# z430/keyword-spotting

Hardware: AMD Instinct MI355X
Metric: 1s 16kHz clips/sec end-to-end (wav->label) (higher is better)
Workload: dtype f32

## Files before the change

keyword-spotting_amd/csrc/kws_dscnn.hip:

```cpp
#include <type_traits>

#include "kws_internal.h"
#include "kws_mfcc_dev.h"
#include "kws_split_mfma.h"

namespace kws {
namespace {


#ifndef KWS_DSCNN_WAVES
#define KWS_DSCNN_WAVES 8
#endif
#ifndef KWS_X_DSCNN_STAMP_TID
#define KWS_X_DSCNN_STAMP_TID 0
#endif
constexpr int NW = KWS_DSCNN_WAVES;
constexpr int NT = NW * 64;
constexpr int TW = 30;

constexpr int P0 = C1_H * C1_W;
constexpr int FEAT_H = 103, FEAT_W = 14;
constexpr int OFF_Z3 = 0, OFF_Z2 = 22976, OFF_Z1 = 0, OFF_Z0 = 9152, OFF_FEAT = 18304;
constexpr int OFF_DWTAB = 38784;
constexpr int OFF_PWB = OFF_DWTAB + 2 * 768;
// ... 69 lines not shown
struct DwPair {
    float4 l[5];
};
template <bool TO_MFMA, int E>
__device__ __forceinline__ float stencil3x3_of_pair(const DwPair& w, float up, float mid, float dn, float mask_l, float mask_r) {
    if constexpr (E == 0)
        return stencil3x3<TO_MFMA>(w.l[0].x, w.l[0].z, w.l[1].x, w.l[1].z, w.l[2].x, w.l[2].z, w.l[3].x, w.l[3].z, w.l[4].x, w.l[4].z, up, mid, dn,
                                   mask_l, mask_r);
    else
        return stencil3x3<TO_MFMA>(w.l[0].y, w.l[0].w, w.l[1].y, w.l[1].w, w.l[2].y, w.l[2].w, w.l[3].y, w.l[3].w, w.l[4].y, w.l[4].w, up, mid, dn,
                                   mask_l, mask_r);
}
__device__ __forceinline__ float half_wave_sum_to_last_lane(float v) {
    v = dpp_shift_add<0x111, 0xf>(v);
    v = dpp_shift_add<0x112, 0xf>(v);
    v = dpp_shift_add<0x114, 0xf>(v);
    v = dpp_shift_add<0x118, 0xf>(v);
    v = dpp_shift_add<0x142, 0xa>(v);
    return v;
}

struct BlockTables {
    float d0, d1, b;
};
__device__ __forceinline__ void fetch_block_tables(const DscnnWeights& w, int n, int tid, BlockTables& r) {
    const float* src = w.dw_w + (n - 1) * CH * 12;
    r.d0 = tid < CH * 12 ? src[tid] : 0.f;
    r.d1 = NT + tid < CH * 12 ? src[NT + tid] : 0.f;
    r.b = tid < CH ? w.pw_b[(n - 1) * CH + tid] : 0.f;
}
__device__ __forceinline__ void store_block_tables(float* lds, int n, int tid, const BlockTables& r, float s_dwb = 1.f, float s_pwb = 1.f,
                                                   float s_dww = 1.f) {
    float* dwtab = lds + OFF_DWTAB + ((n - 1) & 1) * 768;
    if (tid < CH * 12) dwtab[tid] = r.d0 * ((tid % 24) >> 1 == 9 ? s_dwb : s_dww);
    if (NT + tid < CH * 12) dwtab[NT + tid] = r.d1 * (((NT + tid) % 24) >> 1 == 9 ? s_dwb : s_dww);
    if (tid < CH) lds[OFF_PWB + ((n - 1) & 1) * 64 + tid] = r.b * s_pwb;
}
struct PairCtx {
    float s_dww = 1.f;
    float s_dwb = 1.f;
    float s_pwb = 1.f;
    float inv_out = 1.f;
};
__device__ __forceinline__ void cap_units(int& ky, int& sg, int k_w, float bz) {
    sg = ky + k_w;
    const int eb = (int)((__builtin_bit_cast(uint32_t, bz) >> 23) & 0xffu) - 126;
    int limit = 100 - eb;
    limit = limit > 120 ? 120 : limit;
    if (sg > limit) {
        ky -= sg - limit;
        sg = limit;
    }
}
__device__ __forceinline__ void publish_wave_max(float* lds, int set, int wv, int lane, float mx) {
    auto step = [](float m, auto ctrl, auto row_mask) {
        return fmaxf(m, __builtin_bit_cast(float, __builtin_amdgcn_update_dpp(__builtin_bit_cast(int, m), __builtin_bit_cast(int, m), decltype(ctrl)::value,
                                                                              decltype(row_mask)::value, 0xf, false)));
    };
    mx = step(mx, std::integral_constant<int, 0x111>{}, std::integral_constant<int, 0xf>{});
    mx = step(mx, std::integral_constant<int, 0x112>{}, std::integral_constant<int, 0xf>{});
    mx = step(mx, std::integral_constant<int, 0x114>{}, std::integral_constant<int, 0xf>{});
    mx = step(mx, std::integral_constant<int, 0x118>{}, std::integral_constant<int, 0xf>{});
    mx = step(mx, std::integral_constant<int, 0x142>{}, std::integral_constant<int, 0xa>{});
    mx = step(mx, std::integral_constant<int, 0x143>{}, std::integral_constant<int, 0xc>{});
    if (lane == 63) lds[OFF_WMAX + set * NW + wv] = mx;
}
__device__ __forceinline__ float read_stage_max(const float* lds, int set0, int n_sets) {
    static_assert(NW % 4 == 0 && OFF_WMAX % 4 == 0, "the stage maxima are read as float4s");
    float m = 0.f;
    const float4* q = reinterpret_cast<const float4*>(lds + OFF_WMAX + set0 * NW);
    for (int i = 0; i < (NW / 4) * n_sets; ++i) {
        const float4 v = q[i];
        m = fmaxf(fmaxf(m, fmaxf(v.x, v.y)), fmaxf(v.z, v.w));
    }
    return m;
}

template <int NP>
struct PwRing {
    uintx4 ring[2][2][NP];
};
struct PwRegsF32 {
    float wa[2][32];
};
template <int MODE>
using PwOperands = std::conditional_t<(MODE >= 4), PwRing<(MODE == 5 ? 2 : 3)>, PwRegsF32>;
__device__ __forceinline__ void load_pointwise(const DscnnWeights& w, int n, int lane, PwRegsF32& o) {
    const float* pw = w.pw_w + (n - 1) * CH * CH + 8 * (lane >> 5) * CH + (lane & 31);
#pragma unroll
    for (int ct = 0; ct < 2; ++ct)
#pragma unroll
        for (int s = 0; s < 32; ++s) o.wa[ct][s] = pw[(16 * (s >> 3) + (s & 7)) * CH + ct * 32];
}
template <int NP>
__device__ __forceinline__ void load_afrag(const DscnnWeights& w, int n, int m, int lane, uintx4 (&f)[2][NP]) {
    const uintx4* src = reinterpret_cast<const uintx4*>(NP == 2 ? w.pw_pair : w.pw_split) + (size_t)(n - 1) * (2 * 4 * NP * 64) + lane;
#pragma unroll
    for (int ct = 0; ct < 2; ++ct)
#pragma unroll
        for (int p = 0; p < NP; ++p) f[ct][p] = src[((ct * 4 + m) * NP + p) * 64];
}
__device__ __forceinline__ void load_block_head(const DscnnWeights& w, int n, int lane, PwRegsF32& o) { load_pointwise(w, n, lane, o); }
template <int NP>
__device__ __forceinline__ void load_block_head(const DscnnWeights& w, int n, int lane, PwRing<NP>& o) { load_afrag(w, n, 0, lane, o.ring[0]); }

template <bool MFMA>
__device__ __forceinline__ void conv1_phase(const DscnnWeights& w, float* lds, int tid, const float (&a)[50]) {
    const float* featp = lds + OFF_FEAT;
    float* z0 = lds + OFF_Z0;
    if constexpr (MFMA) {
        const int lane = tid & 63, wv = tid >> 6, half = lane >> 5, col = lane & 31;
        const int ct = wv & 1;
        for (int u = wv; u < 10; u += NW) {
            const int pt = u >> 1;
            const int pos = pt * 32 + col;
            const int posc = pos < P0 ? pos : P0 - 1;
            const int oh = posc / C1_W, ow = posc % C1_W;
// ... 118 lines not shown
                __builtin_amdgcn_sched_barrier(0);
            }
            if (kb + 3 < 7) gather(kb + 3, y[nxt]);
            __builtin_amdgcn_sched_barrier(0);
            product(2);
        } else {
#pragma unroll
            for (int i = 0; i < 4; ++i) {
                product(i);
                if (kb + 1 < 7) {
                    const float a0 = y[nxt][2 * i], a1 = y[nxt][2 * i + 1];
                    const float r0 = a0 - top16(a0), r1 = a1 - top16(a1);
                    bf[nxt][0][i] = pack_top16(a0, a1);
                    bf[nxt][1][i] = pack_top16(r0, r1);
                    bf[nxt][NP - 1][i] = pack_top16(r0 - top16(r0), r1 - top16(r1));
                    __builtin_amdgcn_sched_barrier(0);
                }
            }
            product(4);
            if (kb + 3 < 7) gather(kb + 3, y[nxt]);
            __builtin_amdgcn_sched_barrier(0);
            product(5);
        }
        if (DUAL && kb + 2 < 7) {
            load_other(kb + 2);
            __builtin_amdgcn_sched_barrier(0);
        }
    }
    acc += acc2;
    occ += occ2;
    if (pos < p_hi) {
#pragma unroll
        for (int r = 0; r < 16; r += 2) {
            const int co = ct * 32 + row_of(r, half);
            const float v0 = relu(fmaf(w.c1_b[co], sig0, acc[r])), v1 = relu(fmaf(w.c1_b[co + 1], sig0, acc[r + 1]));
            *reinterpret_cast<float2*>(z0 + pidx(co, pos, P0 + 2)) = make_float2(v0, v1);
            if constexpr (PAIR) mx = fmaxf(mx, fmaxf(v0, v1));
            if (DUAL) {
                const int oo = (ct ^ 1) * 32 + row_of(r, half);
                const float u0 = relu(fmaf(w.c1_b[oo], sig0, occ[r])), u1 = relu(fmaf(w.c1_b[oo + 1], sig0, occ[r + 1]));
                *reinterpret_cast<float2*>(z0 + pidx(oo, pos, P0 + 2)) = make_float2(u0, u1);
                if constexpr (PAIR) mx = fmaxf(mx, fmaxf(u0, u1));
            }
        }
    }
}

constexpr int C1W_ROWS = FEAT_H;
constexpr int OFF_C1W8 = OFF_Z1;
constexpr int OFF_C1P2 = OFF_C1W8 + 2 * C1W_ROWS * 3 * 4;
static_assert(OFF_C1P2 + 2 * C1W_ROWS * 3 <= OFF_Z0, "conv1's operand windows live where block 1's output goes later");
static_assert(2 * (C1_W - 1) + 9 < FEAT_W && 2 * (C1_H - 1) + 9 < FEAT_H, "window reach inside the padded map");

__device__ __forceinline__ void conv1_build_windows(float* lds, int tid, float sx, int off_feat = OFF_FEAT) {
    const float* featp = lds + off_feat;
    uint32_t* w8 = reinterpret_cast<uint32_t*>(lds + OFF_C1W8);
    uint32_t* p2 = reinterpret_cast<uint32_t*>(lds + OFF_C1P2);
    for (int i = tid; i < C1W_ROWS * 3; i += NT) {
        const float* src = featp + (i / 3) * FEAT_W + 2 * (i % 3);
        const float y[8] = {src[0], src[1], src[2], src[3], src[4], src[5], src[6], src[7]};
        uintx4 hi, lo;
        split_pair8(y, sx, hi, lo);
        *reinterpret_cast<uintx4*>(w8 + i * 4) = hi;
        *reinterpret_cast<uintx4*>(w8 + (C1W_ROWS * 3 + i) * 4) = lo;
        uint32_t h, l;
        split_pair2(src[8], src[9], sx, h, l);
        p2[i] = h;
        p2[C1W_ROWS * 3 + i] = l;
    }
}

template <bool DUAL>
__device__ __forceinline__ void conv1_unit_pairwin(const DscnnWeights& w, const float* lds, float* z0, int ptile, int ct, int lane,
                                                   const uintx4 (&c1f)[7][2], int p_lo, int p_hi, float sig0, float& mx) {
    const int half = lane >> 5, col = lane & 31;
    const int pos = p_lo + ptile * 32 + col;
    const int posc = pos < p_hi ? pos : p_hi - 1;
    const int oh = posc / C1_W, ow = posc % C1_W;
    const int wi = (2 * oh + 5 * half) * 3 + ow;
    const uintx4* w8 = reinterpret_cast<const uintx4*>(lds + OFF_C1W8) + wi;
    const uint32_t* p2 = reinterpret_cast<const uint32_t*>(lds + OFF_C1P2) + wi;
    const floatx16 zero = {0, 0, 0, 0, 0, 0, 0, 0, 0, 0, 0, 0, 0, 0, 0, 0};
    floatx16 acc = zero, acc2 = zero, occ = zero, occ2 = zero;
    const uintx4* osrc = reinterpret_cast<const uintx4*>(w.c1_pair) + (size_t)(ct ^ 1) * (7 * 2 * 64) + lane;
    uintx4 of[DUAL ? 7 : 1][2];
    if (DUAL) {
#pragma unroll
        for (int kb = 0; kb < 7; ++kb) {
            of[kb][0] = osrc[(kb * 2 + 0) * 64];
            of[kb][1] = osrc[(kb * 2 + 1) * 64];
        }
    }
    float4 cb[4], ob[DUAL ? 4 : 1];
#pragma unroll
    for (int q = 0; q < 4; ++q) {
        cb[q] = *reinterpret_cast<const float4*>(w.c1_b + ct * 32 + 8 * q + 4 * half);
        if (DUAL) ob[DUAL ? q : 0] = *reinterpret_cast<const float4*>(w.c1_b + (ct ^ 1) * 32 + 8 * q + 4 * half);
    }
    uintx4 bq[3][2];
    auto b_load = [&](int kb, uintx4 (&d)[2]) {
        if (kb < 5) {
            d[0] = w8[kb * 3];
            d[1] = w8[kb * 3 + C1W_ROWS * 3];
        } else if (kb == 5) {
#pragma unroll
            for (int i = 0; i < 4; ++i) {
                d[0][i] = p2[i * 3];
                d[1][i] = p2[i * 3 + C1W_ROWS * 3];
            }
        } else {
            d[0] = uintx4{p2[4 * 3], 0u, 0u, 0u};
            d[1] = uintx4{p2[4 * 3 + C1W_ROWS * 3], 0u, 0u, 0u};
        }
    };
    b_load(0, bq[0]);
    b_load(1, bq[1]);
#pragma unroll
    for (int kb = 0; kb < 7; ++kb) {
        if (kb + 2 < 7) b_load(kb + 2, bq[(kb + 2) % 3]);
        const uintx4 &bh = bq[kb % 3][0], &bl = bq[kb % 3][1];
        acc2 = mfma_f16(c1f[kb][0], bl, acc2);
        if (DUAL) occ2 = mfma_f16(of[DUAL ? kb : 0][0], bl, occ2);
        acc = mfma_f16(c1f[kb][1], bh, acc);
        if (DUAL) occ = mfma_f16(of[DUAL ? kb : 0][1], bh, occ);
        acc2 = mfma_f16(c1f[kb][0], bh, acc2);
        if (DUAL) occ2 = mfma_f16(of[DUAL ? kb : 0][0], bh, occ2);
    }
    acc += acc2;
    occ += occ2;
    if (pos < p_hi) {
#pragma unroll
        for (int r = 0; r < 16; r += 2) {
            const int co = ct * 32 + row_of(r, half);
            const float4 b4 = cb[r >> 2];
            const float b0 = (r & 2) ? b4.z : b4.x, b1 = (r & 2) ? b4.w : b4.y;
            const float v0 = relu(fmaf(b0, sig0, acc[r])), v1 = relu(fmaf(b1, sig0, acc[r + 1]));
            *reinterpret_cast<float2*>(z0 + pidx(co, pos, P0 + 2)) = make_float2(v0, v1);
            mx = fmaxf(mx, fmaxf(v0, v1));
            if (DUAL) {
                const int oo = (ct ^ 1) * 32 + row_of(r, half);
                const float4 o4 = ob[DUAL ? (r >> 2) : 0];
                const float c0 = (r & 2) ? o4.z : o4.x, c1 = (r & 2) ? o4.w : o4.y;
                const float u0 = relu(fmaf(c0, sig0, occ[r])), u1 = relu(fmaf(c1, sig0, occ[r + 1]));
                *reinterpret_cast<float2*>(z0 + pidx(oo, pos, P0 + 2)) = make_float2(u0, u1);
                mx = fmaxf(mx, fmaxf(u0, u1));
            }
        }
    }
}

struct PosRange {
    int lo, hi;
};

template <bool RANGED, int NP>
__device__ __forceinline__ void conv1_phase_split(const DscnnWeights& w, float* lds, int tid, const uintx4 (&c1f)[7][NP],
                                                  PosRange rg, float sx = 1.f, float sig0 = 1.f, int off_feat = OFF_FEAT) {
    static_assert(P0 > 4 * 32 && P0 <= 5 * 32 && NW >= 6, "conv1 work split: four dual tiles + one tile in two halves");
    const float* featp = lds + off_feat;
    float* z0 = lds + OFF_Z0;
    const int lane = tid & 63, wv = tid >> 6;
    float mx = 0.f;
    if constexpr (NP == 2) {
        if constexpr (RANGED) {
            const int n_pt = (rg.hi - rg.lo + 31) / 32;
            for (int u = wv; u < 2 * n_pt; u += NW) conv1_unit_pairwin<false>(w, lds, z0, u >> 1, u & 1, lane, c1f, rg.lo, rg.hi, sig0, mx);
        } else if (wv < 4)
            conv1_unit_pairwin<true>(w, lds, z0, wv, wv & 1, lane, c1f, 0, P0, sig0, mx);
        else if (wv < 6)
            conv1_unit_pairwin<false>(w, lds, z0, 4, wv & 1, lane, c1f, 0, P0, sig0, mx);
    } else if constexpr (RANGED) {
        const int n_pt = (rg.hi - rg.lo + 31) / 32;
        for (int u = wv; u < 2 * n_pt; u += NW) conv1_unit_split<false, NP>(w, featp, z0, u >> 1, u & 1, lane, c1f, rg.lo, rg.hi, sx, sig0, mx);
    } else if (wv < 4)
        conv1_unit_split<true, NP>(w, featp, z0, wv, wv & 1, lane, c1f, 0, P0, sx, sig0, mx);
    else if (wv < 6)
        conv1_unit_split<false, NP>(w, featp, z0, 4, wv & 1, lane, c1f, 0, P0, sx, sig0, mx);
    if constexpr (NP == 2) publish_wave_max(lds, 1, wv, lane, mx);
    if (tid < CH) {
        z0[pidx(tid, P0, P0 + 2)] = 0.f;
        z0[pidx(tid, P0 + 1, P0 + 2)] = 0.f;
    }
}

template <int N, int NP>
__device__ __forceinline__ void leftover_partial_unit(float* lds, int lane, int M, const uintx4 (&af)[2][NP]) {
    using G = Blk<N>;
    using L = Leftover<N>;
    const int half = lane >> 5, col = lane & 31;
    const float* dwtab = lds + OFF_DWTAB + G::BUF * 768;
    const float4* dwt4 = reinterpret_cast<const float4*>(dwtab) + half * 24;
    const int pos = L::P0T - 1 + col;
    const bool valid = col >= 1 && col <= TW && pos < G::POUT;
    const int posc = pos < G::POUT ? pos : G::POUT - 1;
    const int h = posc / G::W, x = posc % G::W;
    const float mask_l = x > 0 ? 1.f : 0.f, mask_r = x < G::W - 1 ? 1.f : 0.f;
    int ta[3];
#pragma unroll
    for (int dh = -1; dh <= 1; ++dh) {
        const int o = G::RING ? 1 : 0;
        const int hh = h + dh - o, xx = x - o;
        const bool inside = (unsigned)hh < (unsigned)G::HI && (unsigned)xx < (unsigned)G::WI;
        const bool in_map = (unsigned)(h + dh) < (unsigned)G::H;
        const int a = inside ? hh * G::WI + xx : ((G::RING && in_map) ? G::PIN : G::PIN + 1);
        ta[dh + 1] = G::OFF_IN + pidx(half * 8, a, G::SIN);
    }
    float y[8];
#pragma unroll
    for (int j = 0; j < 8; j += 2) {
        const int cs = 16 * M + j;
        const int o = cs * G::SIN;
        const float2 up = *reinterpret_cast<const float2*>(lds + ta[0] + o);
        const float2 mid = *reinterpret_cast<const float2*>(lds + ta[1] + o);
        const float2 dn = *reinterpret_cast<const float2*>(lds + ta[2] + o);
        DwPair wp;
#pragma unroll
        for (int i = 0; i < 5; ++i) wp.l[i] = dwt4[(cs >> 1) * 6 + i];
        y[j] = stencil3x3_of_pair<false, 0>(wp, up.x, mid.x, dn.x, mask_l, mask_r);
        y[j + 1] = stencil3x3_of_pair<false, 1>(wp, up.y, mid.y, dn.y, mask_l, mask_r);
    }
    floatx16 acc0 = {0, 0, 0, 0, 0, 0, 0, 0, 0, 0, 0, 0, 0, 0, 0, 0}, acc1 = acc0;
    if constexpr (NP == 2) {
        uintx4 bh, bl;
// ... 420 lines not shown
                    "v_add_f32_dpp %8, %8, %8 row_bcast:15 row_mask:0xa bank_mask:0xf\n\t"
                    "v_add_f32_dpp %9, %9, %9 row_bcast:15 row_mask:0xa bank_mask:0xf\n\t"
                    "v_add_f32_dpp %10, %10, %10 row_bcast:15 row_mask:0xa bank_mask:0xf\n\t"
                    "v_add_f32_dpp %11, %11, %11 row_bcast:15 row_mask:0xa bank_mask:0xf\n\t"
                    "v_add_f32_dpp %12, %12, %12 row_bcast:15 row_mask:0xa bank_mask:0xf\n\t"
                    "v_add_f32_dpp %13, %13, %13 row_bcast:15 row_mask:0xa bank_mask:0xf\n\t"
                    "v_add_f32_dpp %14, %14, %14 row_bcast:15 row_mask:0xa bank_mask:0xf\n\t"
                    "v_add_f32_dpp %15, %15, %15 row_bcast:15 row_mask:0xa bank_mask:0xf"
                    : "+v"(q[0]), "+v"(q[1]), "+v"(q[2]), "+v"(q[3]), "+v"(q[4]), "+v"(q[5]), "+v"(q[6]), "+v"(q[7]), "+v"(q[8]), "+v"(q[9]), "+v"(q[10]), "+v"(q[11]), "+v"(q[12]), "+v"(q[13]), "+v"(q[14]), "+v"(q[15]));
            }
            if (col == 31) {
#pragma unroll
                for (int k = 0; k < 32; ++k) poolbuf[wv * CH + (k >> 4) * 32 + row_of(k & 15, half)] = psum[k >> 4][k & 15] * pc.inv_out;
            }
        }
    }
    (void)bias4;
}

template <int NP>
__device__ __forceinline__ void load_conv1_frags(const DscnnWeights& w, int wv, int lane, uintx4 (&c1f)[7][NP]) {
    const uintx4* src = reinterpret_cast<const uintx4*>(NP == 2 ? w.c1_pair : w.c1_split) + (size_t)(wv & 1) * (7 * NP * 64) + lane;
#pragma unroll
    for (int kb = 0; kb < 7; ++kb)
#pragma unroll
        for (int p = 0; p < NP; ++p) c1f[kb][p] = src[(kb * NP + p) * 64];
}

__device__ __forceinline__ int wave_argmax_first(float v, int lane, int C) {
    float m = v;
    m = fmaxf(m, __builtin_bit_cast(float, __builtin_amdgcn_update_dpp(__builtin_bit_cast(int, m), __builtin_bit_cast(int, m), 0x111, 0xf, 0xf, false)));
    m = fmaxf(m, __builtin_bit_cast(float, __builtin_amdgcn_update_dpp(__builtin_bit_cast(int, m), __builtin_bit_cast(int, m), 0x112, 0xf, 0xf, false)));
    m = fmaxf(m, __builtin_bit_cast(float, __builtin_amdgcn_update_dpp(__builtin_bit_cast(int, m), __builtin_bit_cast(int, m), 0x114, 0xf, 0xf, false)));
    m = fmaxf(m, __builtin_bit_cast(float, __builtin_amdgcn_update_dpp(__builtin_bit_cast(int, m), __builtin_bit_cast(int, m), 0x118, 0xf, 0xf, false)));
    m = fmaxf(m, __builtin_bit_cast(float, __builtin_amdgcn_update_dpp(__builtin_bit_cast(int, m), __builtin_bit_cast(int, m), 0x142, 0xa, 0xf, false)));
    m = fmaxf(m, __builtin_bit_cast(float, __builtin_amdgcn_update_dpp(__builtin_bit_cast(int, m), __builtin_bit_cast(int, m), 0x143, 0xc, 0xf, false)));
    const float vmax = __builtin_bit_cast(float, __builtin_amdgcn_readlane(__builtin_bit_cast(int, m), 63));
    const unsigned long long holders = __ballot(lane < C && v == vmax);
    return holders ? __ffsll(holders) - 1 : 0;
}

__device__ __forceinline__ DscnnWeights weights_for_this_clip() {
#if defined(__HIP_DEVICE_COMPILE__)
    using KArg = const __attribute__((address_space(4))) DscnnWeights*;
    KArg p = (KArg)__builtin_amdgcn_kernarg_segment_ptr();
    asm volatile("" : "+s"(p));
    return *p;
#else
    return DscnnWeights{};
#endif
}

template <bool PAIR>
__device__ __forceinline__ void stage_features_persist(float* lds, const float* __restrict__ feat, int clip, int tid) {
    constexpr int ST = STAGE_WAVES * 64;
    constexpr int FV = (IN_T * IN_F + ST - 1) / ST;
    static_assert(2 * STAGE_WAVES == NW, "each staging wavefront zeroes the maximum slot of one other wavefront");
    const int lane = tid & 63, wv = tid >> 6;
    const float* f = feat + (size_t)clip * (IN_T * IN_F);
    float fv[FV];
#pragma unroll
    for (int k = 0; k < FV; ++k) {
        const int i = tid + k * ST;
        fv[k] = i < IN_T * IN_F ? f[i] : 0.f;
    }
    float* featp = lds + OFF_FEAT_P;
    for (int i = tid; i < FEAT_H * FEAT_W; i += ST) {
        const int r = i / FEAT_W - 2, c = i % FEAT_W - 2;
        if (!((unsigned)r < (unsigned)IN_T && (unsigned)c < (unsigned)IN_F)) featp[i] = 0.f;
    }
#pragma unroll
    for (int k = 0; k < FV; ++k) {
        const int i = tid + k * ST;
        if (i < IN_T * IN_F) featp[(i / IN_F + 2) * FEAT_W + (i % IN_F) + 2] = fv[k];
    }
    if constexpr (PAIR) {
        float m = 0.f;
#pragma unroll
        for (int k = 0; k < FV; ++k) m = fmaxf(m, fabsf(fv[k]));
        publish_wave_max(lds, 0, wv, lane, m);
        if (lane == 63) lds[OFF_WMAX + wv + STAGE_WAVES] = 0.f;
    }
}

__device__ __forceinline__ void pool_fc_wave(const DscnnWeights& w, const float* lds, int lane, int clip, float* __restrict__ logits,
                                             int32_t* __restrict__ label, float* __restrict__ a_pool) {
    const int C = w.num_classes;
    float4 fcw[CH / 4];
    float fcb = 0.f;
    const float4* wr = reinterpret_cast<const float4*>(w.fc_w + (lane < C ? lane : 0) * CH);
#pragma unroll
    for (int c = 0; c < CH / 4; ++c) fcw[c] = wr[c];
    if (lane < C) fcb = w.fc_b[lane];
    const float ring_b = w.pw_b[3 * CH + lane];
    constexpr float RING_N = 55.f * 11.f - 53.f * 9.f;
    float s = 0.f;
#pragma unroll
    for (int k = 0; k < NW; ++k) s += lds[OFF_POOLBUF_P + k * CH + lane];
    s = fmaf(RING_N, relu(ring_b), s) * (1.0f / (55.f * 11.f));
    if (a_pool) a_pool[lane] = s;
    float acc = fcb;
#pragma unroll
    for (int c = 0; c < CH / 4; ++c) {
        const float4 a4 = fcw[c];
        acc = fmaf(a4.x, __builtin_bit_cast(float, __builtin_amdgcn_readlane(__builtin_bit_cast(int, s), 4 * c + 0)), acc);
        acc = fmaf(a4.y, __builtin_bit_cast(float, __builtin_amdgcn_readlane(__builtin_bit_cast(int, s), 4 * c + 1)), acc);
        acc = fmaf(a4.z, __builtin_bit_cast(float, __builtin_amdgcn_readlane(__builtin_bit_cast(int, s), 4 * c + 2)), acc);
        acc = fmaf(a4.w, __builtin_bit_cast(float, __builtin_amdgcn_readlane(__builtin_bit_cast(int, s), 4 * c + 3)), acc);
    }
    if (lane < C) logits[(size_t)clip * C + lane] = acc;
    const int idx = wave_argmax_first(lane < C ? acc : -INFINITY, lane, C);
    if (label && lane == 0) label[clip] = idx;
}


template <int MODE, bool DIAG = true, bool PRECONV = false, bool STREAM = false, bool CLUSTER = false, bool PERSIST = false>
__global__ __launch_bounds__(NT) void kws_dscnn_fwd_kernel(DscnnWeights w_arg, const float* __restrict__ feat, int B,
                                                           float* __restrict__ logits, int32_t* __restrict__ label,
                                                           float* __restrict__ act_arg,
                                                           unsigned long long* __restrict__ stamps_arg,
                                                           const int* __restrict__ ring_hops, StreamPush sp) {
    static_assert(!STREAM || (MODE >= 4 && !DIAG && !PRECONV), "the fused push exists for the product paths only");
    static_assert(!PERSIST || ((MODE == 4 || MODE == 5) && !PRECONV && !STREAM), "persistent workgroups: batched product paths only");
    constexpr bool PAIR = MODE == 5;
    constexpr int NP = PAIR ? 2 : 3;
    BlockTables t1_pre{};
    static_assert(!CLUSTER || STREAM, "time-tile clusters exist for the streaming push only");
    float* const act = DIAG ? act_arg : nullptr;
    unsigned long long* const stamps = DIAG ? stamps_arg : nullptr;
    extern __shared__ __attribute__((aligned(16))) float lds[];
    constexpr bool MFMA = MODE != 0;
    const int tid_k = threadIdx.x;
    const int lane_k = tid_k & 63, wv_k = tid_k >> 6;

    const int cl_n = CLUSTER ? sp.cluster : 1;
    int clip = CLUSTER ? (int)blockIdx.x / cl_n : (int)blockIdx.x;
    const int cl_tile = CLUSTER ? (int)blockIdx.x - clip * cl_n : 0;
    if (clip >= B) return;
    const int j0 = Blk<4>::H * cl_tile / cl_n, j1 = Blk<4>::H * (cl_tile + 1) / cl_n;
    auto rows = [&](int lo, int hi, int H, int W) { return PosRange{(lo < 0 ? 0 : lo) * W, (hi > H ? H : hi) * W}; };
    const PosRange rg4 = rows(j0, j1, Blk<4>::H, Blk<4>::W), rg3 = rows(j0 - 2, j1, Blk<3>::H, Blk<3>::W),
                   rg2 = rows(j0 - 4, j1, Blk<2>::H, Blk<2>::W), rg1 = rows(j0 - 6, j1, Blk<1>::H, Blk<1>::W),
                   rg0 = rows(j0 - 7, j1 + 1, C1_H, C1_W);
    int n_stamp = 0;
    auto stamp = [&]() {
        if (stamps && tid_k == KWS_X_DSCNN_STAMP_TID) stamps[(size_t)clip * KWS_DSCNN_STAMPS + n_stamp] = __builtin_amdgcn_s_memtime();
        ++n_stamp;
    };

    constexpr bool SPLIT = MODE >= 4;
    BlockTables t1p{};
    uintx4 c1p[PERSIST ? 7 : 1][NP];
    int prev_clip = -1;
    float* a_prev = nullptr;
    if constexpr (PERSIST) {
        fetch_block_tables(w_arg, 1, tid_k, t1p);
        if (wv_k < STAGE_WAVES) stage_features_persist<PAIR>(lds, feat, clip, tid_k);
        load_conv1_frags(w_arg, wv_k, lane_k, c1p);
        __syncthreads();
    }
    for (;;) {
    const DscnnWeights w = PERSIST ? weights_for_this_clip() : w_arg;
    int tid = tid_k;
    if constexpr (PERSIST) {
        int wv_l = __builtin_amdgcn_readfirstlane(wv_k), lane_l = lane_k;
        asm volatile("" : "+s"(wv_l), "+v"(lane_l));
        tid = (wv_l << 6) | (lane_l & 63);
    }
    const int lane = tid & 63, wv = tid >> 6;
    if constexpr (PERSIST) n_stamp = 0;
    if (stamps && tid == KWS_X_DSCNN_STAMP_TID) stamps[(size_t)clip * KWS_DSCNN_STAMPS + KWS_DSCNN_STAMPS - 2] = __builtin_amdgcn_s_memrealtime();
    stamp();

    PwOperands<MODE> wa;
    int hops_before = 0;
    int kx = 0, ky[5] = {0, 0, 0, 0, 0}, sg[5] = {0, 0, 0, 0, 0};
    if constexpr (PERSIST) {
        if constexpr (PAIR) {
            const float mxf = read_stage_max(lds, 0, 1);
            kx = pow2_exp_for(mxf);
            const float bz0 = (w.c1_abs * mxf + w.c1_bmax) * 1.001f;
            cap_units(kx, sg[0], w.k_c1, bz0);
            const float by1 = (w.dw_abs[0] * bz0 + w.dw_bmax[0]) * 1.001f;
            ky[1] = pow2_exp_for(by1);
            cap_units(ky[1], sg[1], w.k_pw[0], (w.pw_abs[0] * by1 + w.pw_bmax[0]) * 1.001f);
            store_block_tables(lds, 1, tid, t1p, pow2f(ky[1]), pow2f(sg[1]), pow2f(ky[1] - sg[0]));
            conv1_build_windows(lds, tid, pow2f(kx), OFF_FEAT_P);
            __syncthreads();
        } else {
            store_block_tables(lds, 1, tid, t1p);
        }
        stamp();
        conv1_phase_split<false, NP>(w, lds, tid, c1p, rg0, pow2f(kx), pow2f(sg[0]), OFF_FEAT_P);
        if (wv == NW - 1 && prev_clip >= 0) {
            pool_fc_wave(w, lds, lane, prev_clip, logits, label, a_prev);
            if (stamps && lane == 0) stamps[(size_t)prev_clip * KWS_DSCNN_STAMPS + 13] = __builtin_amdgcn_s_memtime();
        }
        load_afrag(w, 1, wv >= 4 ? wv - 4 : 0, lane, wa.ring[0]);
    } else if constexpr (PRECONV) {
        static_assert(!PRECONV || MODE >= 4, "the pre-convolved entry exists for the product (split) path only");
        const float* z = feat + (size_t)clip * (CH * P0);
        fetch_block_tables(w, 1, tid, t1_pre);
        float zmax = 0.f;
        for (int i = tid; i < CH * P0; i += NT) {
            const float v = z[i];
            lds[OFF_Z0 + pidx(i / P0, i % P0, P0 + 2)] = v;
            zmax = fmaxf(zmax, v);
        }
        if (tid < CH) {
            lds[OFF_Z0 + pidx(tid, P0, P0 + 2)] = 0.f;
            lds[OFF_Z0 + pidx(tid, P0 + 1, P0 + 2)] = 0.f;
        }
        if constexpr (PAIR)
            publish_wave_max(lds, 1, wv, lane, zmax);
        else
            store_block_tables(lds, 1, tid, t1_pre);
        if constexpr (Leftover<1>::HAS && (MODE == 4 || MODE == 5) && !CLUSTER)
            load_afrag(w, 1, wv >= 4 ? wv - 4 : 0, lane, wa.ring[0]);
        else
            load_block_head(w, 1, lane, wa);
        stamp();
    } else {
    float* featp = lds + OFF_FEAT;
    const float* f = feat + (size_t)clip * (IN_T * IN_F);
    constexpr int FV = (IN_T * IN_F + NT - 1) / NT;
    float fv[FV];
    int row_new = -1;
    int head;
    if constexpr (STREAM) {
        hops_before = *sp.hops;
        const int K = (sp.p.frame_len + sp.p.frame_step - 1) / sp.p.frame_step;
        head = (((hops_before + 2 - K) % IN_T) + IN_T) % IN_T;
        const int step = sp.p.frame_step;
        const long f_start = (long)step * hops_before + step - (long)((sp.p.frame_len + step - 1) / step) * step;
        if (f_start >= 0) row_new = (int)((((f_start / step) - head) % IN_T + IN_T) % IN_T);
    } else {
        head = ring_hops ? (((*ring_hops + 1 - sp.frames_lag) % IN_T) + IN_T) % IN_T : 0;
    }
#pragma unroll
    for (int k = 0; k < FV; ++k) {
        const int i = tid + k * NT;
        fv[k] = (i < IN_T * IN_F && i / IN_F != row_new) ? f[((i / IN_F + head) % IN_T) * IN_F + i % IN_F] : 0.f;
    }
    BlockTables t1;
    fetch_block_tables(w, 1, tid, t1);
    __builtin_amdgcn_sched_barrier(0);
// ... 121 lines not shown
    if constexpr (PAIR) {
        const float mz = fmaxf(read_stage_max(lds, 2, (Leftover<1>::HAS && KSL_ON) ? 2 : 1) * pow2f(-sg[1]), w.pw_bmax[0]);
        const float bz = (w.pw_abs[1] * ((w.dw_abs[1] * mz + w.dw_bmax[1]) * 1.001f) + w.pw_bmax[1]) * 1.001f;
        const float by = (w.dw_abs[2] * bz + w.dw_bmax[2]) * 1.001f;
        ky[3] = pow2_exp_for(by);
        cap_units(ky[3], sg[3], w.k_pw[2], (w.pw_abs[2] * by + w.pw_bmax[2]) * 1.001f);
        pc.s_dww = pow2f(ky[3] - sg[2]);
        pc.s_dwb = pow2f(ky[3]);
        pc.s_pwb = pow2f(sg[3]);
    }
    block_phase<2, MODE, CLUSTER>(w, lds, tid, wa, nullptr, rg2, pc);
    stamp();
    __syncthreads();
    if constexpr (Leftover<2>::HAS && KSL_ON) {
        leftover_combine<2, PAIR>(lds, tid);
        __syncthreads();
    }
    stamp();
    if (a) {
        const float u = PAIR ? pow2f(-sg[2]) : 1.f;
        for (int i = tid; i < CH * Blk<2>::POUT; i += NT)
            a[i] = lds[OFF_Z2 + pidx(i / Blk<2>::POUT, i % Blk<2>::POUT, Blk<2>::SOUT)] * u;
        a += CH * Blk<2>::POUT;
    }
    if constexpr (PAIR) {
        const float mz = fmaxf(read_stage_max(lds, 0, (Leftover<2>::HAS && KSL_ON) ? 2 : 1) * pow2f(-sg[2]), w.pw_bmax[1]);
        const float bz = (w.pw_abs[2] * ((w.dw_abs[2] * mz + w.dw_bmax[2]) * 1.001f) + w.pw_bmax[2]) * 1.001f;
        const float by = (w.dw_abs[3] * bz + w.dw_bmax[3]) * 1.001f;
        ky[4] = pow2_exp_for(by);
        cap_units(ky[4], sg[4], w.k_pw[3], (w.pw_abs[3] * by + w.pw_bmax[3]) * 1.001f);
        pc.s_dww = pow2f(ky[4] - sg[3]);
        pc.s_dwb = pow2f(ky[4]);
        pc.s_pwb = pow2f(sg[4]);
    }
    block_phase<3, MODE, CLUSTER>(w, lds, tid, wa, nullptr, rg3, pc);
    stamp();
    __syncthreads();
    stamp();
    if (a) {
        const float u = PAIR ? pow2f(-sg[3]) : 1.f;
        for (int i = tid; i < CH * Blk<3>::POUT; i += NT)
            a[i] = lds[OFF_Z3 + pidx(i / Blk<3>::POUT, i % Blk<3>::POUT, Blk<3>::SOUT)] * u;
        a += CH * Blk<3>::POUT;
    }
    if constexpr (PAIR) {
        pc.inv_out = pow2f(-sg[4]);
    }
    block_phase<4, MODE, CLUSTER>(w, lds, tid, wa, a ? a + CH : nullptr, rg4, pc,
                                  PERSIST ? OFF_POOLBUF_P : OFF_POOLBUF);
    stamp();
    if constexpr (PERSIST) {
        const int next = clip + (int)gridDim.x;
        __builtin_amdgcn_sched_barrier(0);
        if (wv < STAGE_WAVES && next < B) stage_features_persist<PAIR>(lds, feat, next, tid);
        stamp();
        load_conv1_frags(w, wv, lane, c1p);
        __syncthreads();
        stamp();
        if (stamps && tid == KWS_X_DSCNN_STAMP_TID) stamps[(size_t)clip * KWS_DSCNN_STAMPS + KWS_DSCNN_STAMPS - 1] = __builtin_amdgcn_s_memrealtime();
        prev_clip = clip;
        a_prev = a;
        clip = next;
        if (clip >= B) break;
        continue;
    }
    const int C = w.num_classes;
    float4 fcw[CH / 4];
    float fcb = 0.f, ring_b = 0.f;
    if (wv == 0 && lane < C) {
        const float4* wr = reinterpret_cast<const float4*>(w.fc_w + lane * CH);
#pragma unroll
        for (int c = 0; c < CH / 4; ++c) fcw[c] = wr[c];
        fcb = w.fc_b[lane];
    }
    if (tid < CH) ring_b = w.pw_b[3 * CH + tid];
    __syncthreads();
    stamp();

    float* pooled = lds + OFF_POOLED;
    constexpr float RING_N = 55.f * 11.f - 53.f * 9.f;
    bool run_fc = true;
    if constexpr (CLUSTER) {
        float* part = sp.cl_part + ((size_t)clip * cl_n + cl_tile) * CH;
        if (tid < CH) {
            float s = 0.f;
#pragma unroll
            for (int k = 0; k < NW; ++k) s += lds[OFF_POOLBUF + k * CH + tid];
            __hip_atomic_store(part + tid, s, __ATOMIC_RELAXED, __HIP_MEMORY_SCOPE_AGENT);
        }
        asm volatile("s_waitcnt vmcnt(0)" ::: "memory");
        __syncthreads();
        int* last_flag = reinterpret_cast<int*>(lds + OFF_POOLED + CH);
        if (tid == 0) {
            const int arrived = atomicAdd(&sp.cl_count[clip], 1);
            *last_flag = arrived == cl_n - 1;
            if (arrived == cl_n - 1) sp.cl_count[clip] = 0;
        }
        __syncthreads();
        run_fc = *last_flag != 0;
        if (run_fc) {
            if (tid < CH) {
                float s = 0.f;
                for (int t = 0; t < cl_n; ++t)
                    s += __hip_atomic_load(sp.cl_part + ((size_t)clip * cl_n + t) * CH + tid, __ATOMIC_RELAXED, __HIP_MEMORY_SCOPE_AGENT);
                pooled[tid] = fmaf(RING_N, relu(ring_b), s) * (1.0f / (55.f * 11.f));
            }
        }
// ... 326 lines not shown
```

Baseline: 7.050 million.

## Build next clip's conv1 windows and block-1 tables during the previous clip's tail

In the persistent kernel, the staging wavefronts now compute the next clip's input maximum, derive the front scale exponents, write the block-1 depthwise and pointwise tables, and build the split conv1 operand windows straight from global memory into a spare region of the Z2 plane. This removes the per-clip table fetch/store, the window build, and one __syncthreads from the head of each clip, and drops the padded feature staging on the pair path. In exchange, the staging waves do more global loads and more arithmetic in the tail, including a redundant per-wave read of the full clip for the max. The change also relies on new LDS overlap invariants, which are asserted statically.

```diff
diff --git a/keyword-spotting_amd/csrc/kws_dscnn.hip b/keyword-spotting_amd/csrc/kws_dscnn.hip
--- a/keyword-spotting_amd/csrc/kws_dscnn.hip
+++ b/keyword-spotting_amd/csrc/kws_dscnn.hip
@@ -145,7 +145,15 @@
         sg = limit;
     }
 }
-__device__ __forceinline__ void publish_wave_max(float* lds, int set, int wv, int lane, float mx) {
+__device__ __forceinline__ void front_scales(const DscnnWeights& w, float mxf, int& kx, int& sg0, int& ky1, int& sg1) {
+    kx = pow2_exp_for(mxf);
+    const float bz0 = (w.c1_abs * mxf + w.c1_bmax) * 1.001f;
+    cap_units(kx, sg0, w.k_c1, bz0);
+    const float by1 = (w.dw_abs[0] * bz0 + w.dw_bmax[0]) * 1.001f;
+    ky1 = pow2_exp_for(by1);
+    cap_units(ky1, sg1, w.k_pw[0], (w.pw_abs[0] * by1 + w.pw_bmax[0]) * 1.001f);
+}
+__device__ __forceinline__ float wave_max_to_last_lane(float mx) {
     auto step = [](float m, auto ctrl, auto row_mask) {
         return fmaxf(m, __builtin_bit_cast(float, __builtin_amdgcn_update_dpp(__builtin_bit_cast(int, m), __builtin_bit_cast(int, m), decltype(ctrl)::value,
                                                                               decltype(row_mask)::value, 0xf, false)));
@@ -156,6 +164,10 @@
     mx = step(mx, std::integral_constant<int, 0x118>{}, std::integral_constant<int, 0xf>{});
     mx = step(mx, std::integral_constant<int, 0x142>{}, std::integral_constant<int, 0xa>{});
     mx = step(mx, std::integral_constant<int, 0x143>{}, std::integral_constant<int, 0xc>{});
+    return mx;
+}
+__device__ __forceinline__ void publish_wave_max(float* lds, int set, int wv, int lane, float mx) {
+    mx = wave_max_to_last_lane(mx);
     if (lane == 63) lds[OFF_WMAX + set * NW + wv] = mx;
 }
 __device__ __forceinline__ float read_stage_max(const float* lds, int set0, int n_sets) {
@@ -380,8 +392,30 @@
 static_assert(OFF_C1P2 + 2 * C1W_ROWS * 3 <= OFF_Z0, "conv1's operand windows live where block 1's output goes later");
 static_assert(2 * (C1_W - 1) + 9 < FEAT_W && 2 * (C1_H - 1) + 9 < FEAT_H, "window reach inside the padded map");
 
-__device__ __forceinline__ void conv1_build_windows(float* lds, int tid, float sx, int off_feat = OFF_FEAT) {
-    const float* featp = lds + off_feat;
+constexpr int C1W_FLOATS = 2 * C1W_ROWS * 3 * 4 + 2 * C1W_ROWS * 3;
+constexpr int OFF_C1W8_P = OFF_POOLBUF_P + NW * CH;
+static_assert(OFF_C1W8_P % 4 == 0 && OFF_C1W8_P >= OFF_POOLBUF_P + NW * CH && OFF_C1W8_P >= OFF_FEAT_P + FEAT_H * FEAT_W,
+              "the next clip's windows are 16-byte aligned and clear of the pool partials (read beside conv1) and the features");
+static_assert(OFF_C1W8_P >= OFF_Z3 + Blk<3>::SOUT * CH && OFF_C1W8_P >= OFF_Z0 + (P0 + 2) * CH,
+              "... of block 4's input (read while they are built) and of conv1's output (written while they are read)");
+static_assert(OFF_C1W8_P + C1W_FLOATS <= OFF_Z2 + Blk<2>::SOUT * CH && OFF_Z2 + Blk<2>::SOUT * CH <= OFF_DWTAB,
+              "... inside the Z2 plane, clear of the table buffers written in the same tail");
+
+__device__ __forceinline__ void conv1_store_window(float* lds, int off_w8, int i, const float (&y)[10], float sx) {
+    uint32_t* w8 = reinterpret_cast<uint32_t*>(lds + off_w8);
+    uint32_t* p2 = w8 + 2 * C1W_ROWS * 3 * 4;
+    const float y8[8] = {y[0], y[1], y[2], y[3], y[4], y[5], y[6], y[7]};
+    uintx4 hi, lo;
+    split_pair8(y8, sx, hi, lo);
+    *reinterpret_cast<uintx4*>(w8 + i * 4) = hi;
+    *reinterpret_cast<uintx4*>(w8 + (C1W_ROWS * 3 + i) * 4) = lo;
+    uint32_t h, l;
+    split_pair2(y[8], y[9], sx, h, l);
+    p2[i] = h;
+    p2[C1W_ROWS * 3 + i] = l;
+}
+__device__ __forceinline__ void conv1_build_windows(float* lds, int tid, float sx) {
+    const float* featp = lds + OFF_FEAT;
     uint32_t* w8 = reinterpret_cast<uint32_t*>(lds + OFF_C1W8);
     uint32_t* p2 = reinterpret_cast<uint32_t*>(lds + OFF_C1P2);
     for (int i = tid; i < C1W_ROWS * 3; i += NT) {
@@ -398,7 +432,7 @@
     }
 }
 
-template <bool DUAL>
+template <bool DUAL, int OFF_W8 = OFF_C1W8>
 __device__ __forceinline__ void conv1_unit_pairwin(const DscnnWeights& w, const float* lds, float* z0, int ptile, int ct, int lane,
                                                    const uintx4 (&c1f)[7][2], int p_lo, int p_hi, float sig0, float& mx) {
     const int half = lane >> 5, col = lane & 31;
@@ -406,8 +440,8 @@
     const int posc = pos < p_hi ? pos : p_hi - 1;
     const int oh = posc / C1_W, ow = posc % C1_W;
     const int wi = (2 * oh + 5 * half) * 3 + ow;
-    const uintx4* w8 = reinterpret_cast<const uintx4*>(lds + OFF_C1W8) + wi;
-    const uint32_t* p2 = reinterpret_cast<const uint32_t*>(lds + OFF_C1P2) + wi;
+    const uintx4* w8 = reinterpret_cast<const uintx4*>(lds + OFF_W8) + wi;
+    const uint32_t* p2 = reinterpret_cast<const uint32_t*>(lds + OFF_W8 + (OFF_C1P2 - OFF_C1W8)) + wi;
     const floatx16 zero = {0, 0, 0, 0, 0, 0, 0, 0, 0, 0, 0, 0, 0, 0, 0, 0};
     floatx16 acc = zero, acc2 = zero, occ = zero, occ2 = zero;
     const uintx4* osrc = reinterpret_cast<const uintx4*>(w.c1_pair) + (size_t)(ct ^ 1) * (7 * 2 * 64) + lane;
@@ -481,7 +515,7 @@
     int lo, hi;
 };
 
-template <bool RANGED, int NP>
+template <bool RANGED, int NP, int OFF_W8 = OFF_C1W8>
 __device__ __forceinline__ void conv1_phase_split(const DscnnWeights& w, float* lds, int tid, const uintx4 (&c1f)[7][NP],
                                                   PosRange rg, float sx = 1.f, float sig0 = 1.f, int off_feat = OFF_FEAT) {
     static_assert(P0 > 4 * 32 && P0 <= 5 * 32 && NW >= 6, "conv1 work split: four dual tiles + one tile in two halves");
@@ -494,9 +528,9 @@
             const int n_pt = (rg.hi - rg.lo + 31) / 32;
             for (int u = wv; u < 2 * n_pt; u += NW) conv1_unit_pairwin<false>(w, lds, z0, u >> 1, u & 1, lane, c1f, rg.lo, rg.hi, sig0, mx);
         } else if (wv < 4)
-            conv1_unit_pairwin<true>(w, lds, z0, wv, wv & 1, lane, c1f, 0, P0, sig0, mx);
+            conv1_unit_pairwin<true, OFF_W8>(w, lds, z0, wv, wv & 1, lane, c1f, 0, P0, sig0, mx);
         else if (wv < 6)
-            conv1_unit_pairwin<false>(w, lds, z0, 4, wv & 1, lane, c1f, 0, P0, sig0, mx);
+            conv1_unit_pairwin<false, OFF_W8>(w, lds, z0, 4, wv & 1, lane, c1f, 0, P0, sig0, mx);
     } else if constexpr (RANGED) {
         const int n_pt = (rg.hi - rg.lo + 31) / 32;
         for (int u = wv; u < 2 * n_pt; u += NW) conv1_unit_split<false, NP>(w, featp, z0, u >> 1, u & 1, lane, c1f, rg.lo, rg.hi, sx, sig0, mx);
@@ -1023,34 +1057,72 @@
 }
 
 template <bool PAIR>
-__device__ __forceinline__ void stage_features_persist(float* lds, const float* __restrict__ feat, int clip, int tid) {
+__device__ __forceinline__ void stage_next_clip(float* lds, const DscnnWeights& w, const float* __restrict__ feat, int clip, int tid) {
     constexpr int ST = STAGE_WAVES * 64;
-    constexpr int FV = (IN_T * IN_F + ST - 1) / ST;
     static_assert(2 * STAGE_WAVES == NW, "each staging wavefront zeroes the maximum slot of one other wavefront");
+    static_assert(CH * 12 == 3 * ST, "three depthwise table entries per staging thread");
     const int lane = tid & 63, wv = tid >> 6;
     const float* f = feat + (size_t)clip * (IN_T * IN_F);
-    float fv[FV];
-#pragma unroll
-    for (int k = 0; k < FV; ++k) {
-        const int i = tid + k * ST;
-        fv[k] = i < IN_T * IN_F ? f[i] : 0.f;
-    }
-    float* featp = lds + OFF_FEAT_P;
-    for (int i = tid; i < FEAT_H * FEAT_W; i += ST) {
-        const int r = i / FEAT_W - 2, c = i % FEAT_W - 2;
-        if (!((unsigned)r < (unsigned)IN_T && (unsigned)c < (unsigned)IN_F)) featp[i] = 0.f;
-    }
-#pragma unroll
-    for (int k = 0; k < FV; ++k) {
-        const int i = tid + k * ST;
-        if (i < IN_T * IN_F) featp[(i / IN_F + 2) * FEAT_W + (i % IN_F) + 2] = fv[k];
-    }
+    float d[3];
+#pragma unroll
+    for (int k = 0; k < 3; ++k) d[k] = w.dw_w[tid + k * ST];
+    const float pb = tid < CH ? w.pw_b[tid] : 0.f;
+    float* dwtab = lds + OFF_DWTAB;
+    auto store_tables = [&](float s_dwb, float s_pwb, float s_dww) {
+#pragma unroll
+        for (int k = 0; k < 3; ++k) dwtab[tid + k * ST] = d[k] * (((tid + k * ST) % 24) >> 1 == 9 ? s_dwb : s_dww);
+        if (tid < CH) lds[OFF_PWB + tid] = pb * s_pwb;
+    };
     if constexpr (PAIR) {
+        constexpr int MV = (IN_T * IN_F + 63) / 64;
+        constexpr int WS = (C1W_ROWS * 3 + ST - 1) / ST;
+        float mv[MV];
+#pragma unroll
+        for (int k = 0; k < MV; ++k) mv[k] = lane + 64 * k < IN_T * IN_F ? f[lane + 64 * k] : 0.f;
+        float y[WS][10];
+#pragma unroll
+        for (int k = 0; k < WS; ++k) {
+            const int i = tid + k * ST;
+            const int r = i / 3 - 2, c0 = 2 * (i % 3) - 2;
+            const bool row_ok = i < C1W_ROWS * 3 && (unsigned)r < (unsigned)IN_T;
+#pragma unroll
+            for (int j = 0; j < 10; ++j) y[k][j] = (row_ok && (unsigned)(c0 + j) < (unsigned)IN_F) ? f[r * IN_F + c0 + j] : 0.f;
+        }
         float m = 0.f;
 #pragma unroll
-        for (int k = 0; k < FV; ++k) m = fmaxf(m, fabsf(fv[k]));
-        publish_wave_max(lds, 0, wv, lane, m);
-        if (lane == 63) lds[OFF_WMAX + wv + STAGE_WAVES] = 0.f;
+        for (int k = 0; k < MV; ++k) m = fmaxf(m, fabsf(mv[k]));
+        m = wave_max_to_last_lane(m);
+        if (lane == 63) {
+            lds[OFF_WMAX + wv] = m;
+            lds[OFF_WMAX + wv + STAGE_WAVES] = 0.f;
+        }
+        const float mxf = __builtin_bit_cast(float, __builtin_amdgcn_readlane(__builtin_bit_cast(int, m), 63));
+        int kx, sg0, ky1, sg1;
+        front_scales(w, mxf, kx, sg0, ky1, sg1);
+        store_tables(pow2f(ky1), pow2f(sg1), pow2f(ky1 - sg0));
+        const float sx = pow2f(kx);
+#pragma unroll
+        for (int k = 0; k < WS; ++k)
+            if (tid + k * ST < C1W_ROWS * 3) conv1_store_window(lds, OFF_C1W8_P, tid + k * ST, y[k], sx);
+    } else {
+        constexpr int FV = (IN_T * IN_F + ST - 1) / ST;
+        float fv[FV];
+#pragma unroll
+        for (int k = 0; k < FV; ++k) {
+            const int i = tid + k * ST;
+            fv[k] = i < IN_T * IN_F ? f[i] : 0.f;
+        }
+        float* featp = lds + OFF_FEAT_P;
+        for (int i = tid; i < FEAT_H * FEAT_W; i += ST) {
+            const int r = i / FEAT_W - 2, c = i % FEAT_W - 2;
+            if (!((unsigned)r < (unsigned)IN_T && (unsigned)c < (unsigned)IN_F)) featp[i] = 0.f;
+        }
+#pragma unroll
+        for (int k = 0; k < FV; ++k) {
+            const int i = tid + k * ST;
+            if (i < IN_T * IN_F) featp[(i / IN_F + 2) * FEAT_W + (i % IN_F) + 2] = fv[k];
+        }
+        store_tables(1.f, 1.f, 1.f);
     }
 }
 
@@ -1120,13 +1192,11 @@
     };
 
     constexpr bool SPLIT = MODE >= 4;
-    BlockTables t1p{};
     uintx4 c1p[PERSIST ? 7 : 1][NP];
     int prev_clip = -1;
     float* a_prev = nullptr;
     if constexpr (PERSIST) {
-        fetch_block_tables(w_arg, 1, tid_k, t1p);
-        if (wv_k < STAGE_WAVES) stage_features_persist<PAIR>(lds, feat, clip, tid_k);
+        if (wv_k < STAGE_WAVES) stage_next_clip<PAIR>(lds, w_arg, feat, clip, tid_k);
         load_conv1_frags(w_arg, wv_k, lane_k, c1p);
         __syncthreads();
     }
@@ -1147,22 +1217,9 @@
     int hops_before = 0;
     int kx = 0, ky[5] = {0, 0, 0, 0, 0}, sg[5] = {0, 0, 0, 0, 0};
     if constexpr (PERSIST) {
-        if constexpr (PAIR) {
-            const float mxf = read_stage_max(lds, 0, 1);
-            kx = pow2_exp_for(mxf);
-            const float bz0 = (w.c1_abs * mxf + w.c1_bmax) * 1.001f;
-            cap_units(kx, sg[0], w.k_c1, bz0);
-            const float by1 = (w.dw_abs[0] * bz0 + w.dw_bmax[0]) * 1.001f;
-            ky[1] = pow2_exp_for(by1);
-            cap_units(ky[1], sg[1], w.k_pw[0], (w.pw_abs[0] * by1 + w.pw_bmax[0]) * 1.001f);
-            store_block_tables(lds, 1, tid, t1p, pow2f(ky[1]), pow2f(sg[1]), pow2f(ky[1] - sg[0]));
-            conv1_build_windows(lds, tid, pow2f(kx), OFF_FEAT_P);
-            __syncthreads();
-        } else {
-            store_block_tables(lds, 1, tid, t1p);
-        }
+        if constexpr (PAIR) front_scales(w, read_stage_max(lds, 0, 1), kx, sg[0], ky[1], sg[1]);
         stamp();
-        conv1_phase_split<false, NP>(w, lds, tid, c1p, rg0, pow2f(kx), pow2f(sg[0]), OFF_FEAT_P);
+        conv1_phase_split<false, NP, OFF_C1W8_P>(w, lds, tid, c1p, rg0, pow2f(kx), pow2f(sg[0]), OFF_FEAT_P);
         if (wv == NW - 1 && prev_clip >= 0) {
             pool_fc_wave(w, lds, lane, prev_clip, logits, label, a_prev);
             if (stamps && lane == 0) stamps[(size_t)prev_clip * KWS_DSCNN_STAMPS + 13] = __builtin_amdgcn_s_memtime();
@@ -1390,7 +1447,7 @@
     if constexpr (PERSIST) {
         const int next = clip + (int)gridDim.x;
         __builtin_amdgcn_sched_barrier(0);
-        if (wv < STAGE_WAVES && next < B) stage_features_persist<PAIR>(lds, feat, next, tid);
+        if (wv < STAGE_WAVES && next < B) stage_next_clip<PAIR>(lds, w, feat, next, tid);
         stamp();
         load_conv1_frags(w, wv, lane, c1p);
         __syncthreads();
```

Result: no change. 7.115 million (median of 6 runs) (+0.9%).
